# Arcadia-Science/arcadia-microscopy-tools

Measured on AMD Instinct MI355X. Metric: fields-of-view/sec (4x2048^2 uint16) end-to-end segment+props, higher is better.
Workload: dtype f64; 1 GPU; configs[2]: synthetic 4-channel 2048x2048 uint16 FOVs, DAPI Gaussian+Otsu+open/close+EDT+peak markers+watershed nuclei (SEEDED relief, seeds_first: marker pixels spread first in raster order, cannot tie; SURVEY A.8's plain -EDT relief with exact ties is reported under sublines.a8_exact) + clear_border/relabel + morphology and 4-channel intensity regionprops; mode=weak scaling, 192 FOVs per GPU per step, streams_per_gpu=4, fovs_per_launch=48, max_cells_per_fov=2048, distinct_fovs_per_gpu=8, resident_in_hbm=True

## Files before the change

arcadia_microscopy_tools_amd/csrc/amt_props.hip:

```cpp
#include "amt_internal.h"
#include "amt_perlabel.h"

#include <vector>

typedef unsigned long long u64;

enum { A_N = 0, A_SY, A_SX, A_SYY, A_SXX, A_SXY, A_C1, A_C2, A_C3, A_NACC };

__global__ void __launch_bounds__(256) rp_init_kernel(u64* __restrict__ acc, int* __restrict__ bbox, size_t nlab,
                                                      const int* __restrict__ src) {
    for (size_t i = (size_t)blockIdx.x * 256 + threadIdx.x; i < nlab; i += (size_t)gridDim.x * 256) {
        if (acc)
            for (int k = 0; k < A_NACC; ++k) acc[i * A_NACC + k] = 0;
        bbox[i * 4 + 0] = src ? src[i * 4 + 0] : 0x7fffffff;
        bbox[i * 4 + 1] = src ? src[i * 4 + 1] : 0x7fffffff;
        bbox[i * 4 + 2] = src ? src[i * 4 + 2] : -1;
        bbox[i * 4 + 3] = src ? src[i * 4 + 3] : -1;
    }
}

__global__ void __launch_bounds__(256) rp_boxes_differ_kernel(const int* __restrict__ a, const int* __restrict__ b, size_t n,
                                                              u64* __restrict__ first) {
    for (size_t i = (size_t)blockIdx.x * 256 + threadIdx.x; i < n; i += (size_t)gridDim.x * 256)
        if (a[i] != b[i]) atomicMin(first, (u64)i);
// ... 438 lines not shown
    if (itable) {
        const unsigned ext = amt_wave_reduce_scatter<8, amt_op_min>(e, lane);
        const u64 cnt = __shfl(red, 0), S = __shfl(red, 4 * (6 + lane)), Q = __shfl(red, 4 * (6 + RP_MAXC + lane));
        const unsigned lo = __shfl(ext, 8 * lane), hi = ~__shfl(ext, 8 * (RP_MAXC + lane));
        if (lane < nc) {
            double* o = itable + (li * C + c0 + lane) * 4;
            if (cnt == 0) {
                o[0] = o[1] = o[2] = o[3] = 0.0;
            } else {
                const double dn = (double)cnt;
                o[0] = (double)S / dn;
                o[1] = (double)hi;
                o[2] = (double)lo;
                const double nv = diff_of_products(cnt, Q, S, S);
                const double var = nv / (dn * dn);
                o[3] = sqrt(var < 0.0 ? 0.0 : var);
            }
        }
    }
}

__global__ void __launch_bounds__(256) rp_heights_kernel(const int* __restrict__ bbox, int* __restrict__ hoff,
                                                         int max_label) {
    const int plane = blockIdx.y;
    for (int l = blockIdx.x * 256 + threadIdx.x; l < max_label; l += gridDim.x * 256) {
        const int* B = bbox + ((size_t)plane * max_label + l) * 4;
        hoff[(size_t)plane * max_label + l] = B[2] >= B[0] ? B[2] - B[0] + 1 : 0;
    }
}

constexpr int HULL_HMAX = 48, HULL_WMAX = 250;

__device__ __forceinline__ void rp_write_convex(double* __restrict__ trow, double convex) {
    const double area = trow[AMT_RP_AREA];
    trow[AMT_RP_AREA_CONVEX] = convex;
    trow[AMT_RP_SOLIDITY] = area > 0.0 ? area / convex : 0.0;
}

__device__ __forceinline__ long long floor_div(long long a, long long b) {
    long long q = a / b;
    return (a % b != 0 && a < 0) ? q - 1 : q;
}
__device__ __forceinline__ long long ceil_div(long long a, long long b) {
    long long q = a / b;
    return (a % b != 0 && a > 0) ? q + 1 : q;
}

template <bool CROWS>
__global__ void __launch_bounds__(64) rp_hull_kernel(const int* __restrict__ bbox, const int* __restrict__ hoff,
                                                     const int* __restrict__ htot, const int2* __restrict__ rows,
                                                     int2* __restrict__ chainL, int2* __restrict__ chainR, size_t cap,
                                                     double* __restrict__ table, int max_label, int skip_h,
                                                     int2* __restrict__ crows) {
    const int plane = blockIdx.y;
    const int l = blockIdx.x * 64 + threadIdx.x;
    if (l >= max_label) return;
    const size_t li = (size_t)plane * max_label + l;
    double* trow = CROWS ? nullptr : table + li * AMT_RP_NCOLS;
    const int miny = bbox[li * 4 + 0], maxy = bbox[li * 4 + 2];
    if (maxy < miny) {
        if (!CROWS && skip_h == 0) trow[AMT_RP_AREA_CONVEX] = 0.0;
        return;
    }
    const int h = maxy - miny + 1;
    if (h <= skip_h && bbox[li * 4 + 3] - bbox[li * 4 + 1] + 1 <= HULL_WMAX) return;
    const size_t off = (size_t)hoff[li];
    if ((size_t)htot[plane] > cap || off + (size_t)h > cap) {
        if (!CROWS) rp_write_convex(trow, __longlong_as_double(0x7ff8000000000000ll));
        return;
    }
    const int2* r = rows + (size_t)plane * cap + off;
    int2* CL = chainL + (size_t)plane * 3 * cap + 3 * off;
    int2* CR = chainR + (size_t)plane * 3 * cap + 3 * off;
    int nl = 0, nr = 0;
    for (int Y = 2 * miny - 1; Y <= 2 * maxy + 1; ++Y) {
        int mn = 0x7fffffff, mx = -0x7fffffff;
        if (Y & 1) {
            int ya = (Y - 1) / 2, yb = (Y + 1) / 2;
            if (Y < 0) {
                ya = -1;
                yb = 0;
            }
            if (ya >= miny && ya <= maxy) {
                int2 e = r[ya - miny];
                if (e.y >= e.x) {
                    mn = min(mn, 2 * e.x);
                    mx = max(mx, 2 * e.y);
                }
            }
            if (yb >= miny && yb <= maxy) {
                int2 e = r[yb - miny];
                if (e.y >= e.x) {
                    mn = min(mn, 2 * e.x);
                    mx = max(mx, 2 * e.y);
                }
            }
        } else {
            int2 e = r[Y / 2 - miny];
            if (e.y >= e.x) {
                mn = 2 * e.x - 1;
                mx = 2 * e.y + 1;
            }
        }
        if (mx < mn) continue;
        while (nl >= 2) {
            int2 p0 = CL[nl - 2], p1 = CL[nl - 1];
            long long cr = (long long)(p1.x - p0.x) * (mn - p0.y) - (long long)(p1.y - p0.y) * (Y - p0.x);
            if (cr <= 0) --nl; else break;
        }
        CL[nl++] = make_int2(Y, mn);
        while (nr >= 2) {
            int2 p0 = CR[nr - 2], p1 = CR[nr - 1];
            long long cr = (long long)(p1.x - p0.x) * (mx - p0.y) - (long long)(p1.y - p0.y) * (Y - p0.x);
            if (cr >= 0) --nr; else break;
        }
        CR[nr++] = make_int2(Y, mx);
    }
    long long count = 0;
    int il = 0, ir = 0;
    for (int y = miny; y <= maxy; ++y) {
        const int Y = 2 * y;
        while (il + 1 < nl && CL[il + 1].x <= Y) ++il;
        while (ir + 1 < nr && CR[ir + 1].x <= Y) ++ir;
        long long xmin, xmax;
        {
            int2 p0 = CL[il];
            if (p0.x == Y || il + 1 >= nl) {
                xmin = ceil_div(p0.y, 2);
            } else {
                int2 p1 = CL[il + 1];
                long long dY = p1.x - p0.x;
                long long num = (long long)p0.y * dY + (long long)(p1.y - p0.y) * (Y - p0.x);
                xmin = ceil_div(num, 2 * dY);
            }
        }
        {
            int2 p0 = CR[ir];
            if (p0.x == Y || ir + 1 >= nr) {
                xmax = floor_div(p0.y, 2);
            } else {
                int2 p1 = CR[ir + 1];
                long long dY = p1.x - p0.x;
                long long num = (long long)p0.y * dY + (long long)(p1.y - p0.y) * (Y - p0.x);
                xmax = floor_div(num, 2 * dY);
            }
        }
        if (CROWS) crows[(size_t)plane * cap + off + (y - miny)] = make_int2((int)xmin, (int)xmax);
        else if (xmax >= xmin) count += xmax - xmin + 1;
    }
    if (!CROWS) rp_write_convex(trow, (double)count);
}

constexpr int HULL_CH = 2 * HULL_HMAX + 1;
__device__ __forceinline__ int floor_div32(int a, int b) {
    const int q = a / b;
    return (a % b != 0 && a < 0) ? q - 1 : q;
}
__device__ __forceinline__ int ceil_div32(int a, int b) {
    const int q = a / b;
    return (a % b != 0 && a > 0) ? q + 1 : q;
}
template <bool CROWS>
__global__ void __launch_bounds__(64) rp_hull_lds_kernel(const int* __restrict__ bbox, const int* __restrict__ hoff,
                                                         const int* __restrict__ htot, const int2* __restrict__ rows,
                                                         size_t cap, double* __restrict__ table, int max_label,
                                                         int2* __restrict__ crows) {
    __shared__ unsigned short s_rows[HULL_HMAX * 32];
    __shared__ unsigned short s_ch[HULL_CH * 64];
    const int plane = blockIdx.y;
    const int lane = threadIdx.x, side = lane & 1, pr = lane >> 1;
    const int l = blockIdx.x * 32 + pr;
    if (l >= max_label) return;
    const size_t li = (size_t)plane * max_label + l;
    double* trow = CROWS ? nullptr : table + li * AMT_RP_NCOLS;
    const int miny = bbox[li * 4 + 0], x0 = bbox[li * 4 + 1], maxy = bbox[li * 4 + 2], x1 = bbox[li * 4 + 3];
    if (maxy < miny) {
        if (!CROWS && side == 0) trow[AMT_RP_AREA_CONVEX] = 0.0;
        return;
    }
    const int h = maxy - miny + 1;
    if (h > HULL_HMAX || x1 - x0 + 1 > HULL_WMAX) return;
    const size_t off = (size_t)hoff[li];
    if ((size_t)htot[plane] > cap || off + (size_t)h > cap) {
        if (!CROWS && side == 0) rp_write_convex(trow, __longlong_as_double(0x7ff8000000000000ll));
        return;
    }
    const int2* r = rows + (size_t)plane * cap + off;
    for (int k0 = side; k0 < h; k0 += 16) {
        int2 e[8];
#pragma unroll
        for (int u = 0; u < 8; ++u) e[u] = r[min(k0 + 2 * u, h - 1)];
#pragma unroll
        for (int u = 0; u < 8; ++u)
            if (k0 + 2 * u < h)
                s_rows[(k0 + 2 * u) * 32 + pr] =
                    e[u].y >= e[u].x ? (unsigned short)((e[u].x - x0) | ((e[u].y - x0) << 8)) : (unsigned short)255;
    }
    __builtin_amdgcn_s_waitcnt(0);
    __builtin_amdgcn_wave_barrier();
    int nc = 0;
    for (int Yr = 0; Yr <= 2 * h; ++Yr) {
        int mn = 0x7fffffff, mx = -1;
        if (!(Yr & 1)) {
            const int ka = (Yr >> 1) - 1, kb = Yr >> 1;
            if (ka >= 0) {
                const unsigned e = s_rows[ka * 32 + pr];
                if ((e >> 8) >= (e & 255)) {
                    mn = min(mn, 2 * (int)(e & 255) + 1);
                    mx = max(mx, 2 * (int)(e >> 8) + 1);
                }
            }
            if (kb < h) {
                const unsigned e = s_rows[kb * 32 + pr];
                if ((e >> 8) >= (e & 255)) {
                    mn = min(mn, 2 * (int)(e & 255) + 1);
                    mx = max(mx, 2 * (int)(e >> 8) + 1);
                }
            }
        } else {
            const unsigned e = s_rows[(Yr >> 1) * 32 + pr];
            if ((e >> 8) >= (e & 255)) {
                mn = 2 * (int)(e & 255);
                mx = 2 * (int)(e >> 8) + 2;
            }
        }
        if (mx < mn) continue;
        const int val = side ? mx : mn;
        while (nc >= 2) {
            const int v0 = s_ch[(nc - 2) * 64 + lane], v1 = s_ch[(nc - 1) * 64 + lane];
            const int cr = ((v1 >> 9) - (v0 >> 9)) * (val - (v0 & 511)) - ((v1 & 511) - (v0 & 511)) * (Yr - (v0 >> 9));
            if (side ? cr >= 0 : cr <= 0) --nc; else break;
        }
        s_ch[(nc++) * 64 + lane] = (unsigned short)((Yr << 9) | val);
    }
    int count = 0;
    int ic = 0;
    for (int k = 0; k < h; ++k) {
        const int Yr = 2 * k + 1;
        while (ic + 1 < nc && (int)(s_ch[(ic + 1) * 64 + lane] >> 9) <= Yr) ++ic;
        int b;
        const int v0 = s_ch[ic * 64 + lane];
        if ((v0 >> 9) == Yr || ic + 1 >= nc) {
            b = side ? floor_div32((v0 & 511) - 1, 2) : ceil_div32((v0 & 511) - 1, 2);
        } else {
            const int v1 = s_ch[(ic + 1) * 64 + lane];
            const int dY = (v1 >> 9) - (v0 >> 9);
            const int num = ((v0 & 511) - 1) * dY + ((v1 & 511) - (v0 & 511)) * (Yr - (v0 >> 9));
            b = side ? floor_div32(num, 2 * dY) : ceil_div32(num, 2 * dY);
        }
        const int other = __shfl_xor(b, 1);
        const int xmin = side ? other : b, xmax = side ? b : other;
        if (CROWS) {
            if (side == 0) crows[(size_t)plane * cap + off + k] = make_int2(xmin + x0, xmax + x0);
        } else if (xmax >= xmin) {
            count += xmax - xmin + 1;
        }
    }
    if (!CROWS && side == 0) rp_write_convex(trow, (double)count);
}

__global__ void __launch_bounds__(256) rp_final_kernel(const u64* __restrict__ acc, const int* __restrict__ bbox,
                                                       double* __restrict__ table, size_t nlab) {
    for (size_t i = (size_t)blockIdx.x * 256 + threadIdx.x; i < nlab; i += (size_t)gridDim.x * 256) {
        const u64* A = acc + i * A_NACC;
        const int* B = bbox + i * 4;
        double* t = table + i * AMT_RP_NCOLS;
        const u64 n = A[A_N];
        if (n == 0) {
            for (int k = 0; k < AMT_RP_NCOLS; ++k)
                if (k != AMT_RP_AREA_CONVEX) t[k] = 0.0;
            continue;
        }
        const double dn = (double)n;
        t[AMT_RP_AREA] = dn;
        t[AMT_RP_CENTROID_Y] = (double)A[A_SY] / dn;
        t[AMT_RP_CENTROID_X] = (double)A[A_SX] / dn;
        t[AMT_RP_BBOX_Y0] = (double)B[0];
        t[AMT_RP_BBOX_X0] = (double)B[1];
        t[AMT_RP_BBOX_Y1] = (double)(B[2] + 1);
        t[AMT_RP_BBOX_X1] = (double)(B[3] + 1);
        const double SQ2 = 1.4142135623730951;
        t[AMT_RP_PERIMETER] = (double)A[A_C1] + (double)A[A_C2] * SQ2 + (double)A[A_C3] * ((1.0 + SQ2) / 2.0);
        const double Nyy = diff_of_products(n, A[A_SYY], A[A_SY], A[A_SY]);
        const double Nxx = diff_of_products(n, A[A_SXX], A[A_SX], A[A_SX]);
        const double Nxy = diff_of_products(n, A[A_SXY], A[A_SX], A[A_SY]);
        const double n2 = dn * dn;
        const double a = Nxx / n2;
        const double c = Nyy / n2;
        const double b = -Nxy / n2;
        const double tr = (a + c) * 0.5;
        const double hd = (a - c) * 0.5;
        const double rad = sqrt(hd * hd + b * b);
        double l1 = tr + rad, l2 = tr - rad;
        l1 = l1 < 0.0 ? 0.0 : l1;
        l2 = l2 < 0.0 ? 0.0 : l2;
        t[AMT_RP_AXIS_MAJOR] = 4.0 * sqrt(l1);
        t[AMT_RP_AXIS_MINOR] = 4.0 * sqrt(l2);
        t[AMT_RP_ECCENTRICITY] = l1 == 0.0 ? 0.0 : sqrt(1.0 - l2 / l1);
        double orient;
        if (Nxx == Nyy) {
            orient = (Nxy > 0.0) ? -0.78539816339744828 : 0.78539816339744828;
        } else {
            orient = 0.5 * atan2(-2.0 * b, c - a);
        }
        t[AMT_RP_ORIENTATION] = orient;
    }
}

extern "C" int amt_regionprops(amt_ctx* ctx, const int32_t* labels, const uint16_t* intensity, int C, double* table_dev,
                               double* itable_dev, int nplanes, int H, int W, int max_label) {
    AMT_REQUIRE(labels && (table_dev || itable_dev) && nplanes >= 0 && H > 0 && W > 0 && max_label >= 0,
                "regionprops: bad arguments");
    AMT_REQUIRE(!intensity == !itable_dev && (!itable_dev || C >= 1),
                "regionprops: the intensity planes (C >= 1) and the intensity table go together");
    AMT_CHECK_OPERANDS("amt_regionprops", amt_in("labels", labels, amt_span(4, nplanes, H, W)),
                       amt_in("intensity", intensity, amt_span(2, nplanes, C, H, W)),
                       amt_out("table_dev", table_dev, amt_span(8, nplanes, max_label, AMT_RP_NCOLS)),
                       amt_out("itable_dev", itable_dev, amt_span(8, nplanes, max_label, C, 4)));
    AMT_TRY(amt_set_device(ctx));
    const bool want_morph = table_dev != nullptr;
    if (nplanes == 0 || max_label == 0) return AMT_OK;
    const size_t n = (size_t)H * W;
    const size_t nlab = (size_t)nplanes * max_label;
    const size_t cap = want_morph ? n : 1;
    amt_scratch s(ctx);
    amt_buf<u64> acc(s, nlab * A_NACC);
    amt_buf<int> bbox(s, nlab * 4);
    amt_buf<int> hoff(s, nlab);
    amt_buf<int> htot(s, nplanes);
    amt_buf<int2> rows(s, (size_t)nplanes * cap);
    amt_buf<int2> chainL(s, (size_t)nplanes * 3 * cap);
    amt_buf<int2> chainR(s, (size_t)nplanes * 3 * cap);
    AMT_TRY(s.commit());
    AMT_TRY(amt_i_label_boxes(ctx, labels, bbox, acc, nplanes, H, W, max_label));
    hipLaunchKernelGGL(rp_heights_kernel, dim3(amt_grid_for(max_label, 256, 256), nplanes), dim3(256), 0, ctx->stream,
                       bbox, hoff, max_label);
    AMT_LAUNCH_CHECK();
    AMT_TRY(amt_scan_excl(ctx, hoff, max_label, (size_t)max_label, htot, nplanes));
    const int groups = intensity ? (C + RP_MAXC - 1) / RP_MAXC : 1;
    for (int g = 0; g < groups; ++g) {
        const int c0 = g * RP_MAXC;
        const int nc = intensity ? ((C - c0) < RP_MAXC ? (C - c0) : RP_MAXC) : 0;
        hipLaunchKernelGGL(rp_label_kernel, dim3(max_label, nplanes), dim3(64), 0, ctx->stream, labels, bbox, hoff, htot,
                           rows, cap, acc, intensity, C, c0, nc, intensity ? itable_dev : (double*)nullptr, H, W,
                           max_label, (want_morph && g == 0) ? 3 : 0);
        AMT_LAUNCH_CHECK();
    }
    if (want_morph) {
        hipLaunchKernelGGL(rp_final_kernel, dim3(amt_grid_for(nlab, 256, 1024)), dim3(256), 0, ctx->stream, acc, bbox,
                           table_dev, nlab);
        AMT_LAUNCH_CHECK();
        const int skip_h = HULL_HMAX;
        hipLaunchKernelGGL(rp_hull_lds_kernel<false>, dim3((max_label + 31) / 32, nplanes), dim3(64), 0, ctx->stream, bbox,
                           hoff, htot, rows, cap, table_dev, max_label, (int2*)nullptr);
        AMT_LAUNCH_CHECK();
        hipLaunchKernelGGL(rp_hull_kernel<false>, dim3((max_label + 63) / 64, nplanes), dim3(64), 0, ctx->stream, bbox,
                           hoff, htot, rows, chainL, chainR, cap, table_dev, max_label, skip_h, (int2*)nullptr);
        AMT_LAUNCH_CHECK();
    }
    return AMT_OK;
}

__global__ void __launch_bounds__(64) rp_intensity_f64_kernel(const int* __restrict__ labels, const int* __restrict__ bbox,
                                                              const double* __restrict__ inten, int C,
                                                              double* __restrict__ itable, int H, int W, int max_label) {
    const int plane = blockIdx.y, l = blockIdx.x, lane = threadIdx.x;
    const size_t li = (size_t)plane * max_label + l;
    const amt_box box = amt_load_box(bbox, li);
    const int y0 = box.y0, x0 = box.x0, y1 = box.y1, x1 = box.x1;
    double* out = itable + li * (size_t)C * 4;
    if (box.absent()) {
        amt_fill_row(out, C * 4, 0.0, lane);
        return;
    }
    const size_t n = (size_t)H * W;
    const int* lab = labels + (size_t)plane * n;
    for (int c = 0; c < C; ++c) {
        const double* img = inten + ((size_t)plane * C + c) * n;
        double s = 0.0, cnt = 0.0, mn = __longlong_as_double(0x7ff0000000000000ll), mx = -mn;
        for (int y = y0; y <= y1; ++y)
            for (int x = x0 + lane; x <= x1; x += 64)
                if (lab[(size_t)y * W + x] == l + 1) {
                    const double v = img[(size_t)y * W + x];
                    s += v;
                    cnt += 1.0;
                    mn = v < mn ? v : mn;
                    mx = v > mx ? v : mx;
                }
        s = amt_wave_sum(s);
        cnt = amt_wave_sum(cnt);
        mn = amt_wave_min(mn);
        mx = amt_wave_max(mx);
        const double mean = s / cnt;
        double q = 0.0;
        for (int y = y0; y <= y1; ++y)
            for (int x = x0 + lane; x <= x1; x += 64)
                if (lab[(size_t)y * W + x] == l + 1) {
                    const double d = img[(size_t)y * W + x] - mean;
                    q += d * d;
                }
        q = amt_wave_sum(q);
// ... 811 lines not shown
```

arcadia_microscopy_tools_amd/csrc/amt_watershed.hip:

```cpp
#include "amt_internal.h"
#include <hip/hip_ext.h>

enum { CLS_NONE = 0, CLS_UNIFORM = 1, CLS_S = 3, CLS_M = 4, CLS_M2 = 5, CLS_L = 6, CLS_X = 7, CLS_G = 9 };
constexpr int WS_NLISTS = CLS_X - CLS_S + 1;
constexpr int WS_CTR = 24;
enum {
    WS_CTR_X = 0,
    WS_CTR_HBM = 7,
    WS_CTR_HASG = 8,
    WS_CTR_WL = 9,
    WS_CTR_NCOMP = 16
};
constexpr int S_PX = 2048, S_NB = 512;
constexpr int M_PX = 4096, M_NB = 512;
constexpr int M2_PX = 8192, M2_NB = 1024;
constexpr int L_PX = 24576, L_NB = 2048;
constexpr int X_PX = 32512, X_NB = 2048;
constexpr int WS_BOX_BLOCKS = 64, WS_BOX_ROWS = 32;

struct comp_row {
    int cmax;
    int mcnt;
    int x0, y0, x1, y1;
    int labmin, labmax;
// ... 1522 lines not shown
}

__global__ void ws_set_flags_kernel(int* f, int n, int v) {
    int i = blockIdx.x * blockDim.x + threadIdx.x;
    if (i < n) f[i] = v;
}

__device__ __forceinline__ int ws_pixel_label(int r, const int* __restrict__ F, const int* __restrict__ ws, size_t base,
                                              size_t i) {
    if (r < 0) return 0;
    const int f = F[base + r];
    return f > 0 ? f : (f == 0 ? ws[base + i] : 0);
}

__global__ void __launch_bounds__(256) ws_final_kernel(const int* __restrict__ L, const int* __restrict__ F,
                                                       const int* __restrict__ ws, const int* __restrict__ map,
                                                       int* __restrict__ out, size_t n, int max_label) {
    const size_t base = (size_t)blockIdx.y * n;
    const int* M = map + (size_t)blockIdx.y * (max_label + 1);
    const unsigned ml = (unsigned)max_label;
    for (size_t i0 = ((size_t)blockIdx.x * 256 + threadIdx.x) * 4; i0 < n; i0 += (size_t)gridDim.x * 1024) {
        if (i0 + 3 < n && ((base + i0) & 3) == 0) {
            const int4 r = *reinterpret_cast<const int4*>(L + base + i0);
            int4 o = make_int4(0, 0, 0, 0);
            if (r.x >= 0 || r.y >= 0 || r.z >= 0 || r.w >= 0) {
                const int fx = r.x >= 0 ? F[base + r.x] : -1, fy = r.y >= 0 ? F[base + r.y] : -1;
                const int fz = r.z >= 0 ? F[base + r.z] : -1, fw = r.w >= 0 ? F[base + r.w] : -1;
                int4 w = make_int4(0, 0, 0, 0);
                if (fx == 0 || fy == 0 || fz == 0 || fw == 0) w = *reinterpret_cast<const int4*>(ws + base + i0);
                const int vx = fx > 0 ? fx : (fx == 0 ? w.x : 0), vy = fy > 0 ? fy : (fy == 0 ? w.y : 0);
                const int vz = fz > 0 ? fz : (fz == 0 ? w.z : 0), vw = fw > 0 ? fw : (fw == 0 ? w.w : 0);
                o.x = (unsigned)(vx - 1) < ml ? M[vx] : 0;
                o.y = (unsigned)(vy - 1) < ml ? M[vy] : 0;
                o.z = (unsigned)(vz - 1) < ml ? M[vz] : 0;
                o.w = (unsigned)(vw - 1) < ml ? M[vw] : 0;
            }
            *reinterpret_cast<int4*>(out + base + i0) = o;
        } else {
            for (size_t i = i0; i < n && i < i0 + 4; ++i) {
                const int v = ws_pixel_label(L[base + i], F, ws, base, i);
                out[base + i] = (unsigned)(v - 1) < ml ? M[v] : 0;
            }
        }
    }
}

struct ws_box_args {
    int* bbox;
    const comp_row* rows;
    const int* ncomp;
    size_t row_stride;
    int2* flist;
    int* fcount;
    int* fbig;
};

__global__ void __launch_bounds__(1024) ws_label_map_kernel(const int* __restrict__ L, const int* __restrict__ F,
                                                            const int* __restrict__ ws, int* __restrict__ present,
                                                            const int* __restrict__ nlabels, int* __restrict__ count_dev,
                                                            int H, int W, int max_label, amt_runtabs rt, ws_box_args bx) {
    __shared__ int s[1024];
    __shared__ int carry;
    __shared__ int nwalk, big;
    const int plane = blockIdx.x;
    const size_t n = (size_t)H * W;
    const size_t base = (size_t)plane * n;
    int* P = present + (size_t)plane * (max_label + 1);
    const int k = nlabels[plane] < max_label ? nlabels[plane] : max_label;
    for (int l = threadIdx.x; l <= max_label; l += 1024) P[l] = (l >= 1 && l <= k) ? 1 : 0;
    __syncthreads();
    const int perim = 2 * W + 2 * H;
    for (int q = threadIdx.x; q < perim; q += 1024) {
        int y, x;
        if (q < W) {
            y = 0;
            x = q;
        } else if (q < 2 * W) {
            y = H - 1;
            x = q - W;
        } else if (q < 2 * W + H) {
            y = q - 2 * W;
            x = 0;
        } else {
            y = q - 2 * W - H;
            x = W - 1;
        }
        const size_t i = (size_t)y * W + x;
        int r;
        if (rt.tbits) {
            const long long ri = amt_rt_px_run(rt, plane, y, x);
            r = ri < 0 ? -1 : amt_rt_run_root(rt, ri, W);
        } else {
            r = L[base + i];
        }
        const int v = ws_pixel_label(r, F, ws, base, i);
        if (v > 0 && v <= max_label) P[v] = 0;
    }
    if (threadIdx.x == 0) carry = 0;
    __syncthreads();
    for (int start = 1; start <= max_label; start += 1024) {
        const int i = start + threadIdx.x;
        const int v = i <= max_label ? P[i] : 0;
        s[threadIdx.x] = v;
        __syncthreads();
        for (int off = 1; off < 1024; off <<= 1) {
            const int t = threadIdx.x >= off ? s[threadIdx.x - off] : 0;
            __syncthreads();
            s[threadIdx.x] += t;
            __syncthreads();
        }
        const int incl = s[threadIdx.x];
        const int c = carry;
        if (i <= max_label) P[i] = v ? c + incl : 0;
        __syncthreads();
        if (threadIdx.x == 1023) carry = c + incl;
        __syncthreads();
    }
    if (threadIdx.x == 0) count_dev[plane] = carry;
    if (!bx.bbox) return;
    int* B = bx.bbox + (size_t)plane * max_label * 4;
    for (int i = threadIdx.x; i < max_label * 4; i += 1024) B[i] = (i & 2) ? -1 : 0x7fffffff;
    if (threadIdx.x == 0) nwalk = 0, big = 0;
    __syncthreads();
    const comp_row* rows = bx.rows + (size_t)plane * bx.row_stride;
    const int fcap = (int)(bx.row_stride / 2);
    int2* fl = bx.flist + (size_t)plane * fcap;
    const int nc = bx.ncomp[plane];
    for (int i = threadIdx.x; i < nc; i += 1024) {
        const comp_row c = rows[i];
        if (c.cls == CLS_UNIFORM) {
            const int m = (unsigned)(c.labmin - 1) < (unsigned)max_label ? P[c.labmin] : 0;
            if (m > 0) {
                int* b = B + (size_t)(m - 1) * 4;
                atomicMin(&b[0], c.y0);
                atomicMin(&b[1], c.x0);
                atomicMax(&b[2], c.y1);
                atomicMax(&b[3], c.x1);
            }
        } else if (c.cls >= CLS_S) {
            const long long area = (long long)(c.x1 - c.x0 + 3) * (c.y1 - c.y0 + 3);
            const int nb = (c.y1 - c.y0) / WS_BOX_ROWS + 1, nch = (c.x1 - c.x0) / 64 + 1;
            const int at = area > X_PX ? fcap : atomicAdd(&nwalk, nb * nch);
            if (area > X_PX || at > fcap - nb * nch) {
                big = 1;
            } else {
                for (int k = 0; k < nb * nch; ++k) fl[at + k] = make_int2(i, (k % nb) | ((k / nb) << 16));
            }
        }
    }
    __syncthreads();
    if (threadIdx.x == 0) bx.fcount[plane] = big ? 0 : nwalk, bx.fbig[plane] = big;
}

__global__ void __launch_bounds__(256) ws_flood_boxes_kernel(const int* __restrict__ labels, ws_box_args bx, int H, int W,
                                                             int max_label) {
    const int lane = threadIdx.x & 63;
    const int plane = blockIdx.y;
    const int cnt = bx.fcount[plane];
    const int* Lp = labels + (size_t)plane * H * W;
    int* B = bx.bbox + (size_t)plane * max_label * 4;
    const comp_row* rows = bx.rows + (size_t)plane * bx.row_stride;
    const int2* fl = bx.flist + (size_t)plane * (bx.row_stride / 2);
    const unsigned ml = (unsigned)max_label;
    constexpr int FQ = 4;
    for (int j = blockIdx.x * 4 + (threadIdx.x >> 6); j < cnt; j += gridDim.x * 4) {
        const int2 it = fl[j];
        const comp_row c = rows[it.x];
        const int ya = c.y0 + (it.y & 0xffff) * WS_BOX_ROWS;
        const int yb = ya + WS_BOX_ROWS - 1 < c.y1 ? ya + WS_BOX_ROWS - 1 : c.y1;
        const int x = c.x0 + (it.y >> 16) * 64 + lane;
        const bool in = x <= c.x1;
        const int xl = in ? x : c.x1;
        auto load = [&](int y) -> int {
            int v = 0;
            if (in && y >= 0 && y < H && y <= yb + 1) v = Lp[(size_t)y * W + xl];
            return (unsigned)(v - 1) < ml ? v : 0;
        };
        int up = load(ya - 1), cur = load(ya);
        for (int y = ya; y <= yb; y += FQ) {
            int nx[FQ];
#pragma unroll
            for (int q = 0; q < FQ; ++q) nx[q] = load(y + 1 + q);
#pragma unroll
            for (int q = 0; q < FQ; ++q) {
                const int yy = y + q;
                if (yy > yb) break;
                const int dn = nx[q];
                const int l = amt_lane_left(cur), r = amt_lane_right(cur);
                const int ul = amt_lane_left(up), ur = amt_lane_right(up);
                const int dl = amt_lane_left(dn), dr = amt_lane_right(dn);
                if (cur) {
                    int* b = B + (size_t)(cur - 1) * 4;
                    const bool head = l != cur, tail = r != cur;
                    if (head && up != cur) atomicMin(&b[0], yy);
                    if (head && dn != cur) atomicMax(&b[2], yy);
                    if (head && ul != cur && dl != cur) atomicMin(&b[1], x);
                    if (tail && ur != cur && dr != cur) atomicMax(&b[3], x);
                }
                up = cur;
                cur = dn;
            }
        }
    }
}

__global__ void __launch_bounds__(256) ws_final_map_kernel(int* __restrict__ Fall, const int* __restrict__ map,
                                                           const int* __restrict__ rootlist, const int* __restrict__ nroots,
                                                           size_t cap, size_t n, int max_label) {
    const int plane = blockIdx.z, shard = plane * gridDim.y + blockIdx.y;
    int* F = Fall + (size_t)plane * n;
    const int* M = map + (size_t)plane * (max_label + 1);
    const int cnt = nroots[shard] < (int)cap ? nroots[shard] : (int)cap;
    const int* lst = rootlist + (size_t)shard * cap;
    for (int k = blockIdx.x * 256 + threadIdx.x; k < cnt; k += gridDim.x * 256) {
        const int t = lst[k], f = F[t];
        F[t] = f > 0 ? ((unsigned)(f - 1) < (unsigned)max_label ? M[f] : 0) : (f == 0 ? -1 : 0);
    }
}

__global__ void __launch_bounds__(256) ws_final_runs_kernel(const unsigned long long* __restrict__ tbits,
                                                            const unsigned short* __restrict__ rtab,
                                                            const int* __restrict__ nruns, const int* __restrict__ Fall,
                                                            const int* __restrict__ wsall, const int* __restrict__ map,
                                                            int* __restrict__ outall, int H, int W, int segs, int trows,
                                                            int ntiles, int max_label) {
    __shared__ int lab_s[4][SR_CAP];
    __shared__ unsigned long long bits_s[4][64];
    __shared__ int off_s[4][64];
    const int lane = threadIdx.x & 63, wv = threadIdx.x >> 6;
    const int t = blockIdx.x * 4 + wv;
    if (t >= ntiles) return;
    const int bx = t % segs, ty = (t / segs) % trows, plane = t / (segs * trows);
    const size_t n = (size_t)H * W;
    const int* F = Fall + (size_t)plane * n;
    const int* ws = wsall + (size_t)plane * n;
    const int* M = map + (size_t)plane * (max_label + 1);
    int* out = outall + (size_t)plane * n;
    const unsigned ml = (unsigned)max_label;
    const int x0 = bx * 64, ty0 = ty * 64;
    const int c4 = (lane & 15) * 4, rsub = lane >> 4;
    const int xg = x0 + c4;
    const int nr = nruns[t];
    if (nr == 0) {
        if (xg < W) {
#pragma unroll 4
            for (int j = 0; j < 16; ++j) {
                const int y = ty0 + rsub + 4 * j;
                if (y < H) *reinterpret_cast<int4*>(out + (size_t)y * W + xg) = make_int4(0, 0, 0, 0);
            }
        }
        return;
    }
    const unsigned long long w = tbits[(size_t)t * 64 + lane];
    const int cnt = __popcll(w & ~(w << 1));
    bits_s[wv][lane] = w;
    off_s[wv][lane] = ccl_wave_incl_scan(cnt, lane) - cnt;
    const bool fast = nr <= SR_CAP;
    if (fast)
        for (int k = lane; k < nr; k += 64) lab_s[wv][k] = F[ccl_rt_root(rtab, (size_t)t, k, ty, bx, W)];
    __builtin_amdgcn_s_waitcnt(0);
    __builtin_amdgcn_wave_barrier();
    if (xg >= W) return;
    constexpr int FQ = 4;
    const int* lb = lab_s[wv];
    auto lab = [&](int k) -> int { return fast ? lb[k] : F[ccl_rt_root(rtab, (size_t)t, k, ty, bx, W)]; };
#pragma unroll
    for (int half = 0; half < 16 / FQ; ++half) {
        int4 o[FQ], f[FQ];
        bool need[FQ];
#pragma unroll
        for (int q = 0; q < FQ; ++q) {
            const int row = rsub + 4 * (half * FQ + q);
            const unsigned long long ww = bits_s[wv][row];
            const unsigned long long hw = ww & ~(ww << 1);
            const unsigned nib = (unsigned)(ww >> c4) & 15u, hnib = (unsigned)(hw >> c4) & 15u;
            o[q] = make_int4(0, 0, 0, 0);
            if (nib) {
                const int k0 = off_s[wv][row] + __popcll(hw & ((1ull << c4) - 1ull)) - 1;
                const int ka = k0 + (int)(hnib & 1u), kb = k0 + __popc(hnib & 3u), kc = k0 + __popc(hnib & 7u), kd = k0 + __popc(hnib);
                const int la = lab(ka < 0 ? 0 : ka), lb2 = lab(kb < 0 ? 0 : kb), lc = lab(kc < 0 ? 0 : kc), ld = lab(kd < 0 ? 0 : kd);
                o[q].x = (nib & 1u) ? la : 0;
                o[q].y = (nib & 2u) ? lb2 : 0;
                o[q].z = (nib & 4u) ? lc : 0;
                o[q].w = (nib & 8u) ? ld : 0;
            }
            need[q] = (o[q].x | o[q].y | o[q].z | o[q].w) < 0;
        }
#pragma unroll
        for (int q = 0; q < FQ; ++q) {
            const int y = ty0 + rsub + 4 * (half * FQ + q);
            f[q] = make_int4(0, 0, 0, 0);
            if (need[q]) f[q] = *reinterpret_cast<const int4*>(ws + (size_t)y * W + xg);
        }
#pragma unroll
        for (int q = 0; q < FQ; ++q) {
            if (need[q]) {
                if (o[q].x < 0) o[q].x = (unsigned)(f[q].x - 1) < ml ? M[f[q].x] : 0;
                if (o[q].y < 0) o[q].y = (unsigned)(f[q].y - 1) < ml ? M[f[q].y] : 0;
                if (o[q].z < 0) o[q].z = (unsigned)(f[q].z - 1) < ml ? M[f[q].z] : 0;
                if (o[q].w < 0) o[q].w = (unsigned)(f[q].w - 1) < ml ? M[f[q].w] : 0;
            }
        }
#pragma unroll
        for (int q = 0; q < FQ; ++q) {
            const int y = ty0 + rsub + 4 * (half * FQ + q);
            if (y < H) *reinterpret_cast<int4*>(out + (size_t)y * W + xg) = o[q];
        }
    }
}

struct ws_fused {
    int32_t* labels = nullptr;
    int32_t* count = nullptr;
    const int32_t* nlabels_dev = nullptr;
    int max_label = 0;
    const int32_t* mk_list = nullptr;
    const int32_t* mk_count = nullptr;
    int mk_cap = 0;
};

struct ws_args {
    amt_ctx* ctx;
    const void* relief;
    bool use_d2;
    const int32_t* markers;
    const uint8_t* mask;
    int32_t* out;
    int nplanes, H, W, seeds_first;
    ws_fused fu;
    ccl_geom g;
    size_t n, row_stride, bstride;
    bool runs;
};
struct ws_bufs {
    int *L, *T, *moff, *boff, *cursor, *mlist, *next, *F, *rootlist, *nroots;
    comp_row* rows;
    int *btot, *mtot, *counters, *wl, *pf_idx, *pf_ctl, *ccl_scratch, *ties, *P;
    int* fctl;
    unsigned long long* tbits;
    unsigned short* rtab;
    int* nruns;
    unsigned short* roff;
    int *rcomp, *head, *tail;
    hp_elem *gheap, *heap;
    int *ncomp, *has_g, *wl_count;
    amt_runtabs rt;
};

static int ws_emulate(amt_ctx* ctx, const void* relief, bool use_d2, const int32_t* markers, const uint8_t* mask, int32_t* out,
                      hp_elem* gheap, const int* run, int nplanes, int H, int W, int conn) {
    const size_t n = (size_t)H * W;
    hipLaunchKernelGGL(ws_global_init_kernel, dim3(amt_grid_for(n, 256, 1024), nplanes), dim3(256), 0, ctx->stream, markers,
                       mask, out, run, n);
    AMT_LAUNCH_CHECK();
    amt_with_bool(use_d2, [&](auto D2) {
// ... 293 lines not shown
```

Before: 17480 FOV/s.

## Register-cache hull chain, use rcp-based division, and aggregate flood-box atomics in LDS

The convex-hull LDS kernel now keeps the top three chain vertices in registers instead of re-reading LDS on every pop. It restructures the row scan to read each row once, and replaces integer floor/ceil division with a float-reciprocal quotient plus a remainder fix-up, guarded by static asserts on value ranges. The watershed flood-boxes kernel gives each wave a small hash table of label bounding boxes in shared memory. Boundary atomics go to LDS first and are flushed to global once per work item, which cuts global atomic traffic at the cost of CAS probing and extra barriers.

```diff
diff --git a/arcadia_microscopy_tools_amd/csrc/amt_props.hip b/arcadia_microscopy_tools_amd/csrc/amt_props.hip
--- a/arcadia_microscopy_tools_amd/csrc/amt_props.hip
+++ b/arcadia_microscopy_tools_amd/csrc/amt_props.hip
@@ -614,13 +614,21 @@
 }
 
 constexpr int HULL_CH = 2 * HULL_HMAX + 1;
-__device__ __forceinline__ int floor_div32(int a, int b) {
-    const int q = a / b;
-    return (a % b != 0 && a < 0) ? q - 1 : q;
-}
-__device__ __forceinline__ int ceil_div32(int a, int b) {
-    const int q = a / b;
-    return (a % b != 0 && a > 0) ? q + 1 : q;
+static_assert(2 * HULL_WMAX < 512 && 2 * HULL_HMAX + 1 < 128, "a chain vertex is (Yr << 9) | Xr in 16 bits");
+static_assert(HULL_WMAX <= 254, "a row is min | max << 8 with 255 | 0 << 8 for an empty one");
+static_assert((2 * HULL_WMAX + 2) * 2 * HULL_HMAX < (1 << 20), "hull_div's dividend stays below 2^20");
+static_assert(4 * HULL_HMAX <= 256, "hull_div's divisor 2 dY");
+__device__ __forceinline__ int hull_div(int n, int d, int& r) {
+    int q = (int)((float)n * __builtin_amdgcn_rcpf((float)d));
+    r = n - q * d;
+    if (r < 0) {
+        --q;
+        r += d;
+    } else if (r >= d) {
+        ++q;
+        r -= d;
+    }
+    return q;
 }
 template <bool CROWS>
 __global__ void __launch_bounds__(64) rp_hull_lds_kernel(const int* __restrict__ bbox, const int* __restrict__ hoff,
@@ -661,54 +669,57 @@
     __builtin_amdgcn_s_waitcnt(0);
     __builtin_amdgcn_wave_barrier();
     int nc = 0;
-    for (int Yr = 0; Yr <= 2 * h; ++Yr) {
-        int mn = 0x7fffffff, mx = -1;
-        if (!(Yr & 1)) {
-            const int ka = (Yr >> 1) - 1, kb = Yr >> 1;
-            if (ka >= 0) {
-                const unsigned e = s_rows[ka * 32 + pr];
-                if ((e >> 8) >= (e & 255)) {
-                    mn = min(mn, 2 * (int)(e & 255) + 1);
-                    mx = max(mx, 2 * (int)(e >> 8) + 1);
-                }
-            }
-            if (kb < h) {
-                const unsigned e = s_rows[kb * 32 + pr];
-                if ((e >> 8) >= (e & 255)) {
-                    mn = min(mn, 2 * (int)(e & 255) + 1);
-                    mx = max(mx, 2 * (int)(e >> 8) + 1);
-                }
-            }
-        } else {
-            const unsigned e = s_rows[(Yr >> 1) * 32 + pr];
-            if ((e >> 8) >= (e & 255)) {
-                mn = 2 * (int)(e & 255);
-                mx = 2 * (int)(e >> 8) + 2;
-            }
-        }
-        if (mx < mn) continue;
-        const int val = side ? mx : mn;
+    int t0 = 0, t1 = 0, t2 = 0;
+    auto feed = [&](int Yr, int val) {
         while (nc >= 2) {
-            const int v0 = s_ch[(nc - 2) * 64 + lane], v1 = s_ch[(nc - 1) * 64 + lane];
-            const int cr = ((v1 >> 9) - (v0 >> 9)) * (val - (v0 & 511)) - ((v1 & 511) - (v0 & 511)) * (Yr - (v0 >> 9));
-            if (side ? cr >= 0 : cr <= 0) --nc; else break;
-        }
-        s_ch[(nc++) * 64 + lane] = (unsigned short)((Yr << 9) | val);
+            const int cr = ((t0 >> 9) - (t1 >> 9)) * (val - (t1 & 511)) - ((t0 & 511) - (t1 & 511)) * (Yr - (t1 >> 9));
+            if (side ? cr >= 0 : cr <= 0) {
+                --nc;
+                t0 = t1;
+                t1 = t2;
+                if (nc >= 3) t2 = s_ch[(nc - 3) * 64 + lane];
+            } else {
+                break;
+            }
+        }
+        const int nv = (Yr << 9) | val;
+        s_ch[nc * 64 + lane] = (unsigned short)nv;
+        t2 = t1;
+        t1 = t0;
+        t0 = nv;
+        ++nc;
+    };
+    auto mine = [&](unsigned e) -> int { return (e >> 8) >= (e & 255) ? (int)(side ? e >> 8 : e & 255) : -1; };
+    int prev = -1, cur = mine(s_rows[pr]);
+    for (int k = 0; k <= h; ++k) {
+        const int next = k + 1 < h ? mine(s_rows[(k + 1) * 32 + pr]) : -1;
+        const int both = side ? max(prev, cur) : (prev < 0 ? cur : cur < 0 ? prev : min(prev, cur));
+        if (both >= 0) feed(2 * k, 2 * both + 1);
+        if (cur >= 0) feed(2 * k + 1, 2 * cur + 2 * side);
+        prev = cur;
+        cur = next;
     }
     int count = 0;
     int ic = 0;
+    int c0 = s_ch[lane], c1 = s_ch[min(1, nc - 1) * 64 + lane], c2 = s_ch[min(2, nc - 1) * 64 + lane];
     for (int k = 0; k < h; ++k) {
         const int Yr = 2 * k + 1;
-        while (ic + 1 < nc && (int)(s_ch[(ic + 1) * 64 + lane] >> 9) <= Yr) ++ic;
+        while (ic + 1 < nc && (c1 >> 9) <= Yr) {
+            ++ic;
+            c0 = c1;
+            c1 = c2;
+            c2 = s_ch[min(ic + 2, nc - 1) * 64 + lane];
+        }
+        const int v0 = c0, v1 = c1;
         int b;
-        const int v0 = s_ch[ic * 64 + lane];
         if ((v0 >> 9) == Yr || ic + 1 >= nc) {
-            b = side ? floor_div32((v0 & 511) - 1, 2) : ceil_div32((v0 & 511) - 1, 2);
+            b = ((v0 & 511) - side) >> 1;
         } else {
-            const int v1 = s_ch[(ic + 1) * 64 + lane];
             const int dY = (v1 >> 9) - (v0 >> 9);
             const int num = ((v0 & 511) - 1) * dY + ((v1 & 511) - (v0 & 511)) * (Yr - (v0 >> 9));
-            b = side ? floor_div32(num, 2 * dY) : ceil_div32(num, 2 * dY);
+            int r;
+            const int q = hull_div(num + 2 * dY, 2 * dY, r) - 1;
+            b = side ? q : q + (r != 0);
         }
         const int other = __shfl_xor(b, 1);
         const int xmin = side ? other : b, xmax = side ? b : other;
diff --git a/arcadia_microscopy_tools_amd/csrc/amt_watershed.hip b/arcadia_microscopy_tools_amd/csrc/amt_watershed.hip
--- a/arcadia_microscopy_tools_amd/csrc/amt_watershed.hip
+++ b/arcadia_microscopy_tools_amd/csrc/amt_watershed.hip
@@ -1698,8 +1698,11 @@
     if (threadIdx.x == 0) bx.fcount[plane] = big ? 0 : nwalk, bx.fbig[plane] = big;
 }
 
+constexpr int WS_BOX_SLOTS = 16;
 __global__ void __launch_bounds__(256) ws_flood_boxes_kernel(const int* __restrict__ labels, ws_box_args bx, int H, int W,
                                                              int max_label) {
+    __shared__ int s_key[4][WS_BOX_SLOTS];
+    __shared__ int s_box[4][WS_BOX_SLOTS][4];
     const int lane = threadIdx.x & 63;
     const int plane = blockIdx.y;
     const int cnt = bx.fcount[plane];
@@ -1709,6 +1712,14 @@
     const int2* fl = bx.flist + (size_t)plane * (bx.row_stride / 2);
     const unsigned ml = (unsigned)max_label;
     constexpr int FQ = 4;
+    int* key = s_key[threadIdx.x >> 6];
+    int(*box)[4] = s_box[threadIdx.x >> 6];
+    if (lane < WS_BOX_SLOTS) {
+        key[lane] = 0;
+        box[lane][0] = box[lane][1] = 0x7fffffff;
+        box[lane][2] = box[lane][3] = -1;
+    }
+    __builtin_amdgcn_wave_barrier();
     for (int j = blockIdx.x * 4 + (threadIdx.x >> 6); j < cnt; j += gridDim.x * 4) {
         const int2 it = fl[j];
         const comp_row c = rows[it.x];
@@ -1722,6 +1733,7 @@
             if (in && y >= 0 && y < H && y <= yb + 1) v = Lp[(size_t)y * W + xl];
             return (unsigned)(v - 1) < ml ? v : 0;
         };
+        int known = 0, slot = -1;
         int up = load(ya - 1), cur = load(ya);
         for (int y = ya; y <= yb; y += FQ) {
             int nx[FQ];
@@ -1735,18 +1747,57 @@
                 const int l = amt_lane_left(cur), r = amt_lane_right(cur);
                 const int ul = amt_lane_left(up), ur = amt_lane_right(up);
                 const int dl = amt_lane_left(dn), dr = amt_lane_right(dn);
-                if (cur) {
-                    int* b = B + (size_t)(cur - 1) * 4;
-                    const bool head = l != cur, tail = r != cur;
-                    if (head && up != cur) atomicMin(&b[0], yy);
-                    if (head && dn != cur) atomicMax(&b[2], yy);
-                    if (head && ul != cur && dl != cur) atomicMin(&b[1], x);
-                    if (tail && ur != cur && dr != cur) atomicMax(&b[3], x);
+                const bool head = cur && l != cur, tail = cur && r != cur;
+                const bool q0 = head && up != cur, q2 = head && dn != cur;
+                const bool q1 = head && ul != cur && dl != cur, q3 = tail && ur != cur && dr != cur;
+                if (q0 || q1 || q2 || q3) {
+                    if (cur != known) {
+                        known = cur;
+                        slot = -1;
+                        int s = cur & (WS_BOX_SLOTS - 1);
+                        for (int t = 0; t < WS_BOX_SLOTS; ++t) {
+                            const int was = atomicCAS(&key[s], 0, cur);
+                            if (was == 0 || was == cur) {
+                                slot = s;
+                                break;
+                            }
+                            s = (s + 1) & (WS_BOX_SLOTS - 1);
+                        }
+                    }
+                    if (slot >= 0) {
+                        int* b = box[slot];
+                        if (q0) atomicMin(&b[0], yy);
+                        if (q2) atomicMax(&b[2], yy);
+                        if (q1) atomicMin(&b[1], x);
+                        if (q3) atomicMax(&b[3], x);
+                    } else {
+                        int* b = B + (size_t)(cur - 1) * 4;
+                        if (q0) atomicMin(&b[0], yy);
+                        if (q2) atomicMax(&b[2], yy);
+                        if (q1) atomicMin(&b[1], x);
+                        if (q3) atomicMax(&b[3], x);
+                    }
                 }
                 up = cur;
                 cur = dn;
             }
         }
+        __builtin_amdgcn_wave_barrier();
+        if (lane < WS_BOX_SLOTS) {
+            const int k = key[lane];
+            if (k) {
+                const int y0 = box[lane][0], x0 = box[lane][1], y1 = box[lane][2], x1 = box[lane][3];
+                int* b = B + (size_t)(k - 1) * 4;
+                if (y0 != 0x7fffffff) atomicMin(&b[0], y0);
+                if (x0 != 0x7fffffff) atomicMin(&b[1], x0);
+                if (y1 >= 0) atomicMax(&b[2], y1);
+                if (x1 >= 0) atomicMax(&b[3], x1);
+                key[lane] = 0;
+                box[lane][0] = box[lane][1] = 0x7fffffff;
+                box[lane][2] = box[lane][3] = -1;
+            }
+        }
+        __builtin_amdgcn_wave_barrier();
     }
 }
 
```

New measurement: 17500 FOV/s, median of 3. About the same (+0.1%).
